# Ryo1011gd/ParticleMethod_FSI

Measured on AMD Instinct MI355X. Metric: particle-steps/sec + achieved HBM GB/s, dam-break, 1/2/4/8 MI355X, higher is better.
Workload: dtype f64; 1 GPU; d1m: 3-D dam break (SURVEY 8d D1M, BASELINE configs[1]), 1397200 particles, ~1397200 per GPU; particles=1397200, dim=3, module=dam, parallelism=single

## Files before the change

### include/mph_gpu.h

```cpp
#ifndef MPH_GPU_H_INCLUDED
#define MPH_GPU_H_INCLUDED

#include <stddef.h>

#ifdef __cplusplus
extern "C" {
#endif

#define MPH_TYPE_COUNT 6
#define MPH_MAX_NEIGHBOR_COUNT 512
#define MPH_ABI_VERSION 6

typedef enum MphModule {
    MPH_MODULE_BAR = 0,
    MPH_MODULE_DAM = 1,
    MPH_MODULE_TUREK_HRON = 2,
    MPH_MODULE_ROLLING1 = 3,
    MPH_MODULE_HYDROELASTIC = 4,
    MPH_MODULE_NONE = 5
} MphModule;

typedef enum MphWallMotion {
    MPH_WALL_RIGID = 0,
    MPH_WALL_ROLLING = 1
// ... 228 lines not shown
    mph_host_exchange_fn host_fn;
    void* host_user;
    int n_glob;
    const int* ids;
    const double* cuts;
} MphSlabOptions;
int mph_create_slab(MphCtx** ctx, const MphConfig* cfg, int n, const int* property, const double* pos,
                    const double* pos0, const double* vel, int device, const MphSlabOptions* opt);
int mph_slab_window(const MphConfig* cfg, int rank, int nranks, int axis, const double* cuts, double* out2);
int mph_dist_selftest(int device);
int mph_dist_info(const MphCtx* ctx, int* out8);
int mph_dist_overlap(const MphCtx* ctx, double* out5);
int mph_list_stats(MphCtx* ctx, double* mean, int* max);
int mph_list_layout(MphCtx* ctx, long long out6[6]);
int mph_idle_wall_stats(MphCtx* ctx, long long out2[2]);
int mph_neighbor_rows(MphCtx* ctx, int first, int count, int* counts, int* ids, long long ids_cap);
int mph_owned_count(const MphCtx* ctx);
int mph_owned_ids(MphCtx* ctx, int* out_ids);
int mph_slab_bounds(const MphConfig* cfg, int rank, int nranks, int axis, const double* cuts, double* out3);
int mph_slab_owner(const MphConfig* cfg, int nranks, int axis, const double* cuts, double c);

#ifdef __cplusplus
}
#endif
#endif
```

### particlemethod_fsi_amd/csrc/mph_ctx.hip

```cpp
#include <hip/hip_runtime.h>

#include <algorithm>
#include <chrono>
#include <cmath>
#include <cstdio>
#include <cstdlib>
#include <cstring>
#include <map>
#include <memory>
#include <string>
#include <vector>

#include "mph_dist.h"
#include "mph_env.h"
#include "mph_rows.h"

using namespace mph;

namespace mph {

int ctx_fail(MphCtx* c, int code, const std::string& msg)
{
    if (c) c->err = msg;
    return code;
// ... 43 lines not shown
    MPH_HIP_OK(c, hipStreamSynchronize(c->stream));
    for (hipGraphExec_t* g : {&c->graph1, &c->graph1t, &c->graph8})
        if (*g) {
            MPH_HIP_OK(c, hipGraphExecDestroy(*g));
            *g = nullptr;
        }
    return MPH_OK;
}

void ctx_fill_launch(MphCtx* c)
{
    Launch& L = c->L;
    set_uniforms(c->P);
    if (env_int("MPH_LIST_FULL", 0) == 1) c->P.rlf = 3.0e38f;
    c->lazy_walls = !c->dist && env_int("MPH_LAZY_WALLS", 1) != 0;
    L.P = &c->P;
    L.stream = c->stream;
    L.xcd_bal_min = env_is("MPH_XCD_BAL_MIN", "") ? (1 << 20) : env_int("MPH_XCD_BAL_MIN", 1 << 20);
    L.S = &c->Sd;
}

int virial_full_lists(MphCtx* c)
{
    if (c->P.rlf >= 3.0e38f) return MPH_OK;
    DevParams Pf = c->P;
    Pf.rlf = 3.0e38f;
    Launch L = c->L;
    L.P = &Pf;
    L.xcd_bal_min = 0x7fffffff;
    launch_neighbors(L);
    MPH_HIP_OK(c, hipGetLastError());
    return MPH_OK;
}
}

namespace {

void enqueue_step(const Launch& L, bool last, hipEvent_t* ev = nullptr)
{
    if (ev) (void)hipEventRecord(ev[0], L.stream);
    Launch La = L;
    La.lazy = !last && L.cmap && !L.mon;
    launch_sort(La, 1);
    if (!last) {
        La.dens_a = La.vstrain = La.divp = nullptr;
        if (!L.P->surface) La.gx = La.gy = La.gz = La.pa = nullptr;
    }
    if (ev) {
        launch_neighbors(La);
        (void)hipEventRecord(ev[1], L.stream);
        launch_pass_a(La);
    } else {
        launch_search_pass_a(La);
    }
    if (last) {
        launch_pass_b(L);
    } else {
// ... 1107 lines not shown
    MPH_HIP_OK(c, hipSetDevice(c->device));
    MPH_HIP_OK(c, hipStreamSynchronize(c->stream));
    unsigned long long steps = 0;
    std::vector<unsigned> seg(kXcdSegs);
    const char* st = reinterpret_cast<const char*>(c->L.st);
    MPH_HIP_OK(c, hipMemcpy(&steps, st + offsetof(DevState, lazy_steps), sizeof(steps), hipMemcpyDeviceToHost));
    MPH_HIP_OK(c, hipMemcpy(seg.data(), st + offsetof(DevState, idle_waves), sizeof(unsigned) * kXcdSegs,
                            hipMemcpyDeviceToHost));
    long long idle = 0;
    for (unsigned v : seg) idle += v;
    out[0] = idle;
    out[1] = (long long)steps;
    return MPH_OK;
}

int mph_neighbor_rows(MphCtx* c, int first, int count, int* counts, int* ids, long long ids_cap)
{
    if (!c || first < 0 || count < 0 || !counts || (!ids && ids_cap > 0)) return MPH_ERR_ARG;
    MPH_CK(ctx_flush(c));
    if (c->dist) return ctx_fail(c, MPH_ERR_UNSUPPORTED, "mph_neighbor_rows: single contexts only");
    if ((long long)first + count > c->n) return ctx_fail(c, MPH_ERR_ARG, "mph_neighbor_rows: range past the particle count");
    if (!count) return 0;
    MPH_HIP_OK(c, hipSetDevice(c->device));
    const int n = c->n;
    if (c->P.rlf < 3.0e38f)
        return ctx_fail(c, MPH_ERR_UNSUPPORTED, "mph_neighbor_rows: the lists keep only the pairs within the passes' "
                                            "radius (create the context with MPH_LIST_FULL=1 for the reference's lists)");
    std::vector<int> id(n), nv(n);
    MPH_HIP_OK(c, hipMemcpy(id.data(), c->L.A.id, sizeof(int) * n, hipMemcpyDeviceToHost));
    MPH_HIP_OK(c, hipMemcpy(nv.data(), c->L.nbcount, sizeof(int) * n, hipMemcpyDeviceToHost));
// ... 240 lines not shown
```

### particlemethod_fsi_amd/csrc/mph_kernels.h

```cpp
#pragma once

#include <hip/hip_runtime.h>

#include "mph_params.h"

namespace mph {

struct StructDev {
    int* orig = nullptr;
    int* slot_of = nullptr;
    int* bidx = nullptr;
    int n_own = 0;
    int n_inner = 0;
    int wo = 0, wi = 0;
    int* ocnt = nullptr;
    int* icnt = nullptr;
    int* eo_nb = nullptr;
    int* ei_nb = nullptr;
    double4* wx0 = nullptr;
    double* L = nullptr;
    double2* lame = nullptr;
    double* inv_rho = nullptr;
    int* clamp = nullptr;
    double4* x0 = nullptr;
// ... 55 lines not shown
    const DevTables* T = nullptr;
    DevState* st = nullptr;
    hipStream_t stream = nullptr;
    Profiler* prof = nullptr;
    Soa A, B;
    int* dst_of = nullptr;
    int *key = nullptr, *slot = nullptr, *tmp = nullptr, *cnt = nullptr, *start = nullptr, *bsum = nullptr;
    int *nbr = nullptr, *ncount = nullptr, *nbcount = nullptr;
    unsigned long long *lhdr = nullptr, *lgap = nullptr;
    int* wface = nullptr;
    VSrc vsrc;
    int xcd_bal_min = 1 << 20;
    unsigned char* cmap = nullptr;
    int cmap_bytes = 0;
    bool lazy = false;
    double *pres = nullptr, *gx = nullptr, *gy = nullptr, *gz = nullptr, *pa = nullptr;
    double *dens_a = nullptr, *vstrain = nullptr, *divp = nullptr;
    double4 *fpart = nullptr;
    double4 *rec = nullptr;
    double4 *force = nullptr, *acc = nullptr;
    const StructDev* S = nullptr;
    const MonitorDev* mon = nullptr;
};

struct SampleDev {
    double origin[3], spacing[3];
    int count[3];
    int tile[3];
    int tiles[3];
    int mask;
// ... 51 lines not shown
```

### particlemethod_fsi_amd/csrc/mph_params.h

```cpp
#pragma once
#include <cmath>

#include <cstddef>
#include <cstdint>

#include "../../include/mph_gpu.h"


namespace mph {

constexpr int kTypes = MPH_TYPE_COUNT;
constexpr int kMaxNeighbor = MPH_MAX_NEIGHBOR_COUNT;
constexpr int kTile = 64;
constexpr int kAlignRows = 128;
constexpr int kMaxJumps = 6;
#ifndef MPH_TILE_EXTRA
#define MPH_TILE_EXTRA kAlignRows
#endif
constexpr int kTileRows = kMaxNeighbor + MPH_TILE_EXTRA;
#ifndef MPH_TILE_PAD
#define MPH_TILE_PAD 1
#endif
constexpr int kTileStride = kTile * (kTileRows + MPH_TILE_PAD);
#if defined(__HIPCC__)
// ... 65 lines not shown
    double ratio[kTypes][kTypes];
    double mu_ij[kTypes][kTypes];
    double cofa[kTypes];
    double mass[kTypes], inv_mass[kTypes], density[kTypes], inv_density[kTypes];
    double bulk[kTypes], bulk_visc[kTypes];
    double wall_rot[kTypes][3][3];
    double wall_omega[kTypes][3];
    double wall_vel[kTypes][3];
    double rc2_lo, rc2_hi;
    double rc2_trim;
    double cwid[3];
    double rg_r2g;
    double cref[3];
    float rc2f_lo, rc2f_hi;
    float rlf;
};

inline void set_uniforms(DevParams& P)
{
    P.rc2_lo = P.rc2 * (1.0 - 1e-10);
    P.rc2_hi = P.rc2 * (1.0 + 1e-10);
    P.rc2_trim = P.rc2 * (1.0 + 4e-6);
    for (int d = 0; d < 3; ++d) P.cwid[d] = 1.0 / P.ginv[d];
    P.rg_r2g = P.rg / P.r2g;
    double hwm = 0.0;
    for (int d = 0; d < 3; ++d) {
        P.cref[d] = P.dmin[d] + P.hw[d];
        hwm = P.hw[d] > hwm ? P.hw[d] : hwm;
    }
    const double rc = std::sqrt(P.rc2);
    const double delta = 2.0 * (2.0 * 1.7320508 * hwm * 1.1920929e-7 / rc) + 4.0e-6;
    P.rc2f_lo = (float)(P.rc2 * (1.0 - delta));
    P.rc2f_hi = (float)(P.rc2 * (1.0 + delta));
    const double rmax = std::fmax(std::fmax(P.ra, P.rg), std::fmax(P.rp, P.rv));
    P.rlf = (float)(rmax * rmax * (1.0 + delta));
}

constexpr int kCoarseShift = 2;
#if defined(__HIPCC__)
__host__ __device__
#endif
constexpr inline int coarse_cells(int g) { return (g + (1 << kCoarseShift) - 1) >> kCoarseShift; }
inline size_t coarse_map_bytes(const int gc[3])
{
    const size_t b = (size_t)coarse_cells(gc[0]) * coarse_cells(gc[1]) * coarse_cells(gc[2]);
    return (b + 15) & ~(size_t)15;
}

constexpr int kXcdSegs = 4096;

struct DevState {
// ... 4 lines not shown
    double wall_rot[kTypes][3][3];
    int overflow;
    int pad0;
    int seam_occ[2];
    int seam_step;
    int seam_pad;
    int seg_work[kXcdSegs];
    int xcd_frac[9];
    int xcd_pad[3];
    unsigned long long lazy_steps;
    unsigned idle_waves[kXcdSegs];
    int seg_lwork[kXcdSegs];
    int seg_swork[kXcdSegs];
    int xcd_sfrac[9];
    int xcd_spad[3];
};
constexpr size_t kStateHead = offsetof(DevState, seg_work);

#if defined(__HIPCC__)
#define MPH_HD __host__ __device__
#else
#define MPH_HD
#endif

MPH_HD inline int jump_count(unsigned long long hdr) { return (int)(hdr >> 56); }
MPH_HD inline int gap_begin(unsigned long long gap, int k) { return (int)((gap >> (8 * k)) & 0xff); }
MPH_HD inline int gap_end(unsigned long long hdr, int k) { return (int)((hdr >> (8 * k)) & 0xff); }

#ifndef MPH_PA_EQR
#define MPH_PA_EQR 1
// ... 74 lines not shown
```

### particlemethod_fsi_amd/csrc/mph_passes.hip

```cpp
#include <cstdio>
#include <cstdlib>
#include <type_traits>

#include "mph_list.h"

namespace mph {

__device__ __forceinline__ void own_velocity(const Soa& A, int i, double& vx, double& vy, double& vz)
{
    const double2 b = A.p6[3 * (size_t)i + 1], c = A.p6[3 * (size_t)i + 2];
    vx = b.y; vy = c.x; vz = c.y;
}


struct PassA {
    double da = 0.0, g0 = 0.0, g1 = 0.0, g2 = 0.0, vs = 0.0, dv = 0.0;
    double s0 = 0.0, s1 = 0.0, s2 = 0.0, v0 = 0.0, v1 = 0.0, v2 = 0.0;
};

template <bool FORCE, bool EQR = false>
__device__ __forceinline__ void pass_a_term(const DevParams& P, const double* s_ratio, const double* s_mu, int ti,
                                            int tj, bool solid, double q0, double q1, double q2, double r2,
                                            double dvx, double dvy, double dvz, PassA& o)
{
#pragma clang fp contract(off)
    double r, ir;
    rsqrt_pair(r2, r, ir);
    const double dot = fma(dvz, q2, fma(dvy, q1, dvx * q0));
    if (EQR) {
        if (r2 <= P.rp2) {
            const double t = r * P.inv_rp;
            const double omt = 1.0 - t;
            const double omt2 = omt * omt;
            const double u = (P.cdp * omt) * ir;
            o.vs = fma(P.cp, omt2, o.vs);
            o.dv = fma(-dot, u, o.dv);
            const bool strict = r2 < P.rp2;
            if (FORCE && strict && !(solid && dev_is_struct(tj))) {
                const double c = u * P.vol;
                o.s0 = fma(c, q0, o.s0);
                o.s1 = fma(c, q1, o.s1);
                o.s2 = fma(c, q2, o.s2);
            }
            if (!solid) {
                const double ratio = s_ratio[ti * kTypes + tj];
                o.da = fma(ratio, (P.ca * t) * omt2, o.da);
                const double w = (ratio * (P.cg * omt2)) * P.rg_r2g;
                o.g0 = fma(q0, w, o.g0);
                o.g1 = fma(q1, w, o.g1);
                o.g2 = fma(q2, w, o.g2);
                if (FORCE && strict) {
                    const double c = ((s_mu[ti * kTypes + tj] * omt) * dot) * ((ir * ir) * ir);
                    o.v0 = fma(c, q0, o.v0);
                    o.v1 = fma(c, q1, o.v1);
                    o.v2 = fma(c, q2, o.v2);
                }
            }
        }
        return;
    }
    if (r2 <= P.rp2) {
        const double omt = 1.0 - r * P.inv_rp;
        const double u = (P.cdp * omt) * ir;
        o.vs = fma(P.cp * omt, omt, o.vs);
        o.dv = fma(-dot, u, o.dv);
        if (FORCE && r2 < P.rp2 && !(solid && dev_is_struct(tj))) {
            const double c = u * P.vol;
            o.s0 = fma(c, q0, o.s0);
            o.s1 = fma(c, q1, o.s1);
            o.s2 = fma(c, q2, o.s2);
        }
    }
    if (!solid) {
        const double ratio = s_ratio[ti * kTypes + tj];
        if (r2 <= P.ra2) {
            const double t = r * P.inv_ra;
            const double omt = 1.0 - t;
            o.da = fma(ratio, ((P.ca * t) * omt) * omt, o.da);
        }
        if (r2 <= P.rg2) {
            const double omt = 1.0 - r * P.inv_rg;
            const double w = (ratio * ((P.cg * omt) * omt)) * P.rg_r2g;
            o.g0 = fma(q0, w, o.g0);
            o.g1 = fma(q1, w, o.g1);
            o.g2 = fma(q2, w, o.g2);
        }
        if (FORCE && r2 < P.rv2) {
            const double c = ((s_mu[ti * kTypes + tj] * (1.0 - r * P.inv_rv)) * dot) * ((ir * ir) * ir);
            o.v0 = fma(c, q0, o.v0);
            o.v1 = fma(c, q1, o.v1);
            o.v2 = fma(c, q2, o.v2);
        }
    }
}

struct PassAOut {
    double *pres, *gx, *gy, *gz, *pa, *dens_a, *vstrain, *divp;
    double4 *fpart, *rec;
};

// ... 38 lines not shown
template <int U, typename Bits>
__device__ __forceinline__ void list_batch(const NbrList& NL, Bits bits_of, int k0, int end,
                                           bool (&ok)[U], int (&jj)[U], int (&TT)[U])
{
    int e[U];
#pragma unroll
    for (int u = 0; u < U; ++u) nbr_at(NL, k0 + u < end ? k0 + u : end - 1, e[u], TT[u]);
    const unsigned bits = bits_of();
#pragma unroll
    for (int u = 0; u < U; ++u) {
        ok[u] = (bits & (1u << u)) != 0;
        jj[u] = e[u];
    }
}

template <bool FAST, int DIM, bool EQR, int U = MPH_UA>
__device__ __forceinline__ void pass_a_loop(const DevParams& P, const double* s_ratio, const double* s_mu,
                                            const Soa& A,
                                            NbrList NL, bool plain, const unsigned* lm, int end, int ti,
                                            bool solid, double xi, double yi, double zi, double vxi, double vyi,
                                            double vzi, PassA& o)
{
    const __amdgpu_buffer_rsrc_t p6r = sized_rsrc(A.p6, (unsigned)P.n * 48u);
    for (int k0 = 0; k0 < end; k0 += U) {
        int jj[U];
        double X[U], Y[U], Z[U], VX[U], VY[U], VZ[U];
        int TT[U];
        bool ok[U];
        list_batch<U>(NL, [&] { return plain ? bit_range(0, end - k0) : row_bits_lds(lm, k0, end); }, k0, end,
                      ok, jj, TT);
#pragma unroll
        for (int u = 0; u < U; ++u) {
            const unsigned off = ok[u] ? (unsigned)jj[u] * 48u : kGatherOob;
            const double2 a = buf_ld16(p6r, off), b = buf_ld16(p6r, off + 16u), c = buf_ld16(p6r, off + 32u);
            X[u] = a.x; Y[u] = a.y; Z[u] = b.x;
            VX[u] = b.y; VY[u] = c.x; VZ[u] = c.y;
        }
#pragma unroll
        for (int u = 0; u < U; ++u) {
            asm volatile("" ::"v"(X[u]), "v"(Y[u]), "v"(Z[u]), "v"(VX[u]), "v"(VY[u]), "v"(VZ[u]));
            if (!ok[u]) continue;
            const double q0 = image_exact<FAST>(X[u] - xi, P.dw[0], P.hw[0], P.w075[0]);
            const double q1 = image_exact<FAST>(Y[u] - yi, P.dw[1], P.hw[1], P.w075[1]);
            const double q2 = image_exact<FAST || DIM == 2>(Z[u] - zi, P.dw[2], P.hw[2], P.w075[2]);
            pass_a_term<true, EQR>(P, s_ratio, s_mu, ti, TT[u], solid, q0, q1, q2, r2_exact(q0, q1, q2),
                                   VX[u] - vxi, VY[u] - vyi, VZ[u] - vzi, o);
        }
    }
}

#ifndef MPH_PA_WPE
#define MPH_PA_WPE 4
#endif
#if MPH_PA_WPE
#define MPH_PA_ATTR __attribute__((amdgpu_waves_per_eu(MPH_PA_WPE)))
#else
#define MPH_PA_ATTR
#endif
template <int DIM>
__global__ __launch_bounds__(MPH_LB) MPH_PA_ATTR void k_pass_a(DevParams P, const DevTables* __restrict__ T, Soa A,
                                                const int* __restrict__ nbr,
                                                const int* __restrict__ ncount,
                                                const unsigned long long* __restrict__ lhdr,
                                                const unsigned long long* __restrict__ lgap, PassAOut pout,
                                                const DevState* __restrict__ st,
                                                unsigned char* __restrict__ cmap, int cmap_bytes)
{
    const int n = dev_n(P);
    if (cmap)
        for (int q = blockIdx.x * MPH_LB + threadIdx.x; q * 16 < cmap_bytes; q += gridDim.x * MPH_LB)
            reinterpret_cast<int4*>(cmap)[q] = make_int4(0, 0, 0, 0);
    const int lb = list_block(st, n, MPH_PASS_A_REV);
    if (lb < 0) return;
    __shared__ double s_ratio[kTypes * kTypes];
    __shared__ double s_mu[kTypes * kTypes];
    if (threadIdx.x < kTypes * kTypes) {
        s_ratio[threadIdx.x] = T->ratio[threadIdx.x];
        s_mu[threadIdx.x] = T->mu_ij[threadIdx.x] * (-P.cvis * P.cdv * P.vol);
    }
    __syncthreads();
    const int i = lb * blockDim.x + threadIdx.x;
    const bool live = i < n;
    const int ii = live ? i : n - 1;
// ... 9 lines not shown
    if (!own) return;
    double vxi, vyi, vzi;
    own_velocity(A, i, vxi, vyi, vzi);
    const int ti = A.type[i];
    const bool solid = dev_is_struct(ti);
    const int end = ncount[i] < kTileRows ? ncount[i] : kTileRows;
    __shared__ unsigned s_mask[kWB][kTile * kMaskWords];
    unsigned* lm = &s_mask[threadIdx.x >> 6][(threadIdx.x & 63) * kMaskWords];
    const unsigned long long hdr = wave_hdr(lhdr, i);
    const bool plain = (hdr >> 56) == 0;
    if (!plain) mask_to_lds(lm, row_mask(hdr, lgap, i, end));
    const NbrList NL = nbr_list(nbr, i);
    PassA o;
    const bool eqr = pass_a_equal_radii(P);
    if (fast && eqr)
        pass_a_loop<true, DIM, true>(P, s_ratio, s_mu, A, NL, plain, lm, end, ti, solid, xi, yi, zi, vxi, vyi, vzi, o);
    else if (fast)
        pass_a_loop<true, DIM, false>(P, s_ratio, s_mu, A, NL, plain, lm, end, ti, solid, xi, yi, zi, vxi, vyi, vzi, o);
    else
        pass_a_loop<false, DIM, false>(P, s_ratio, s_mu, A, NL, plain, lm, end, ti, solid, xi, yi, zi, vxi, vyi, vzi, o);
    pass_a_finish(P, T, ti, i, o, pout, xi, yi, zi);
}


template <bool FAST, bool SURF, int DIM>
__device__ __forceinline__ void pass_b_term(const DevParams& P, const double* s_ratio, const double* gx,
                                            const double* gy, const double* gz, const double* pa, int j, int tj,
                                            double X, double Y, double Z, double PJ, int ti, bool solid,
                                            double xi, double yi, double zi, double gxi, double gyi, double gzi,
                                            double pai, double ai, double dscale, double cpv, double& f0,
                                            double& f1, double& f2)
{
    if (solid && dev_is_struct(tj)) return;
    const double q0 = image_exact<FAST>(X - xi, P.dw[0], P.hw[0], P.w075[0]);
    const double q1 = image_exact<FAST>(Y - yi, P.dw[1], P.hw[1], P.w075[1]);
// ... 260 lines not shown
#pragma unroll
        for (int v = 0; v < 3; ++v) o[3 * u + v] = S[u][v];
    vpres[i] = DIM == 2 ? -1.0 / 2.0 * (S[0][0] + S[1][1]) : -1.0 / 3.0 * (S[0][0] + S[1][1] + S[2][2]);
}


static PassAOut pass_a_out(const Launch& L)
{
    return PassAOut{L.pres, L.gx, L.gy, L.gz, L.pa, L.dens_a, L.vstrain, L.divp, L.fpart, L.rec};
}

void launch_pass_a(const Launch& L)
{
    const DevParams& P = *L.P;
    if (P.n == 0) return;
    by_dim(P.dim, [&](auto D) {
        launch(L.prof, "pass_a", L.stream, k_pass_a<decltype(D)::value>,
               dim3(list_grid(P.n, L.lazy && P.n >= L.xcd_bal_min)), dim3(MPH_LB), P, L.T,
               L.A, L.nbr, L.ncount, L.lhdr, L.lgap, pass_a_out(L), L.st, L.lazy ? L.cmap : nullptr, L.cmap_bytes);
    });
}

void launch_search_pass_a(const Launch& L)
{
    launch_neighbors(L);
    launch_pass_a(L);
}

static StructHook struct_hook(const Launch& L)
{
    StructHook h{};
    if (L.P->n_struct > 0 && L.S && L.S->slot_of) {
        h.slot_of = L.S->slot_of;
        h.sx = L.S->x;
        h.sv = L.S->v;
// ... 40 lines not shown
```

### particlemethod_fsi_amd/csrc/mph_search.hip

```cpp
#include "mph_list.h"

#ifndef MPH_SB
#define MPH_SB 2
#endif
#ifndef MPH_LDS_CAP
#define MPH_LDS_CAP 176
#endif

namespace mph {

__device__ __forceinline__ void start_load2(__amdgpu_buffer_rsrc_t r, unsigned ob, unsigned oe, int& b, int& e)
{
    asm volatile("s_nop 4\n\tbuffer_load_dword %0, %2, %4, 0 offen\n\tbuffer_load_dword %1, %3, %4, 0 offen"
                 : "=&v"(b), "=&v"(e) : "v"(ob), "v"(oe), "s"(r) : "memory");
}
__device__ __forceinline__ void start_landed(int& a, int& b) { asm volatile("" : "+v"(a), "+v"(b)); }

__host__ __device__ constexpr int stage_d(int cap, int sb) { return (cap + sb + 2 + 1) & ~1; }
__host__ __device__ constexpr int stage_t(int cap, int sb) { return (cap + sb + 8 + 3) & ~3; }
__host__ __device__ constexpr int stage_words(int cap, int sb) { return 3 * stage_d(cap, sb) + stage_t(cap, sb) / 2; }


template <int DIM, int PERM> struct CellAxes {
    static constexpr int A0 = DIM == 3 ? order_axis(PERM, 0) : 0;
// ... 99 lines not shown
                    const double q0 = image_exact<false>(xs[u] - xi, P.dw[0], P.hw[0], P.w075[0]);
                    const double q1 = image_exact<false>(ys[u] - yi, P.dw[1], P.hw[1], P.w075[1]);
                    const double q2 = image_exact<DIM == 2>(zs[u] - zi, P.dw[2], P.hw[2], P.w075[2]);
                    const bool a = r2_exact(q0, q1, q2) <= P.rc2;
                    if (a && j < je && j != i) {
                        if (cnt < kMaxNeighbor) out[ell_slot(cnt, 0)] = nbr_entry(j, A.type[j]);
                        ++cnt;
                    }
                }
            }
        }
    }
    return cnt;
}

template <int DIM, int PERM, int SB = MPH_SB, int CAP = MPH_LDS_CAP>
__device__ __forceinline__ int scan_candidates_lds(const DevParams& P, const Soa& A, const int* start,
                                                   int i, bool act, double xi, double yi, double zi,
                                                   int cx, int cy, int cz, int* out, double* sx, int* stored,
                                                   unsigned long long* lgap, unsigned long long* lhdr)
{
    constexpr int kCap32 = stage_words(CAP, SB) / 2 - SB - 1;
    const int lane = threadIdx.x & 63;
    const unsigned long long tb = (unsigned long long)(out - lane);
    const unsigned tlo = __builtin_amdgcn_readfirstlane((unsigned)tb);
    const unsigned thi = __builtin_amdgcn_readfirstlane((unsigned)(tb >> 32));
    const __amdgpu_buffer_rsrc_t tile_rsrc = __builtin_amdgcn_make_buffer_rsrc(
        reinterpret_cast<void*>(((unsigned long long)thi << 32) | tlo), 0, kTile * kTileRows * (int)sizeof(int),
        0x00020000);
    const double lo2 = P.rc2_lo, hi2 = P.rc2_hi;
    using X = CellAxes<DIM, PERM>;
    constexpr int NCOL = DIM == 3 ? kGroups * kGroups : kGroups;
    const int cc[3] = {cx, cy, cz};
    const int cca = cc[X::A2];
    const double cw0 = P.cwid[X::A0], cw1 = P.cwid[X::A1];
    const double uu[3] = {grid_offset(xi, P.corg[0], P.dw[0]), grid_offset(yi, P.corg[1], P.dw[1]),
                          DIM == 3 ? grid_offset(zi, P.corg[2], P.dw[2]) : 0.0};
    const double ua = uu[X::A2];
    const double ginva = P.ginv[X::A2];
    constexpr float kDn = 1.0f - 1.0f / (1 << 20), kUp = 1.0f + 1.0f / (1 << 19);
    constexpr float kBias = 32.0f;
    const float rcm2f = act ? (float)P.rc2_trim * kUp : -1.0f;
    float gx2f = 0.0f;
    const int c0l = cc[X::A0], c1l = DIM == 3 ? cc[X::A1] : 0;
    const float cw0f = (float)cw0, cw1f = (float)cw1;
    const float f0 = (float)(uu[X::A0] - c0l * cw0), f1 = DIM == 3 ? (float)(uu[X::A1] - c1l * cw1) : 0.0f;
    const float mu0 = cw0f * (1.0f / (1 << 20)), mu1 = cw1f * (1.0f / (1 << 20));
    const float g0p = f0 + mu0, g0m = (cw0f - f0) + mu0, g1p = f1 + mu1, g1m = (cw1f - f1) + mu1;
    const float ginvaf = (float)ginva;
    const float caf = (float)(ua * ginva - (double)cca);
    const float cal = (caf - 1e-3f) + kBias, cah = (caf + 1e-3f) + kBias;
    const float rgf = kUp * ginvaf;
    const int rowbase = (DIM == 3 ? (c0l * P.gc[X::A1] + c1l) * P.gc[X::A2] : c0l * P.gc[1]) + cca - (int)kBias;
    const int sa = P.sa;
    const __amdgpu_buffer_rsrc_t srs = arr_rsrc(start);
    auto gap32 = [](int d, float cwf, float gp, float gm) {
        if (d == 0) return 0.0f;
// ... 113 lines not shown
            const float lof = P.rc2f_lo, hif = P.rc2f_hi;
            auto test32 = [&](auto self_tag) {
                constexpr bool SELF = decltype(self_tag)::value;
                for (int j0 = jb; j0 < je; j0 += SB) {
                    float4 r[SB];
#pragma unroll
                    for (int u = 0; u < SB; ++u) r[u] = s4[j0 - lbase + u];
#pragma unroll
                    for (int u = 0; u < SB; ++u) {
                        const int j = j0 + u;
                        const float dx = r[u].x - xf, dy = r[u].y - yf, dz = r[u].z - zf;
                        const float r2f = fmaf(dx, dx, fmaf(dy, dy, dz * dz));
                        bool live = true;
                        if (u > 0) live = j < je;
                        if (SELF) live = live & (j != i);
                        const bool le_lo = r2f <= lof, le_hi = r2f <= hif;
                        bool a = live & le_lo;
                        const unsigned long long mband = __builtin_amdgcn_ballot_w64(le_hi) &
                                                         ~__builtin_amdgcn_ballot_w64(le_lo) &
                                                         __builtin_amdgcn_ballot_w64(live);
                        if (mband) {
                            if (__builtin_amdgcn_inverse_ballot_w64(mband)) {
                                int jj = j;
                                asm volatile("" : "+v"(jj));
                                const double ddx = A.x[jj] - xi, ddy = A.y[jj] - yi, ddz = A.z[jj] - zi;
                                const double r2a = fma(ddx, ddx, fma(ddy, ddy, ddz * ddz));
                                const bool in = r2a <= lo2;
                                a = in;
                                if ((r2a <= hi2) != in) a = accept_band(P, ddx, ddy, ddz);
                            }
// ... 47 lines not shown
    return soff_total(soff);
}

__device__ __forceinline__ void slab_wave_flag(const DevParams& P, const Soa& A, int i, int n, int* wface)
{
    if (P.slab_axis < 0 || !wface) return;
    const bool live = i < n;
    const int ii = live ? i : n - 1;
    const bool own = live && A.id[ii] >= 0;
    const double c = P.slab_axis == 0 ? A.x[ii] : (P.slab_axis == 1 ? A.y[ii] : A.z[ii]);
    const bool inner = c - P.slab_lo > P.slab_h && P.slab_hi - c > P.slab_h;
    const bool face = !__all(!own || inner);
    if ((threadIdx.x & 63) == 0) wface[i >> 6] = face ? 1 : 0;
}

template <int DIM>
__device__ __forceinline__ bool wave_idle_walls(const DevParams& P, const Soa& A, const unsigned char* cmap,
                                                DevState* st, int* ncount, int* nbcount,
                                                unsigned long long* lhdr, int i, int n)
{
    static_assert(kContigReach <= kReach, "the box is widened by kReach on every axis");
    static_assert(2 * kReach < 2 << kCoarseShift, "a lane's box spans at most 3 coarse cells per axis");
    const int tile = __builtin_amdgcn_readfirstlane(i >> 6);
    if (tile * kTile >= n) return false;
    const bool live = i < n;
    int ii = live ? i : n - 1;
    asm volatile("" : "+v"(ii));
    if (!__all(!live || dev_is_wall(A.type[ii]))) return false;
    const double xi = A.x[ii], yi = A.y[ii], zi = A.z[ii];
    if (!wave_search_interior(P, st, live, xi, yi, zi)) return false;
    const int cx = cell_axis(xi, P.corg[0], P.dw[0], P.ginv[0], P.gc[0]);
// ... 3 lines not shown
    const int ay = max(cy - kReach, 0) >> kCoarseShift, by = min(cy + kReach, P.gc[1] - 1) >> kCoarseShift;
    const int az = DIM == 3 ? max(cz - kReach, 0) >> kCoarseShift : 0;
    const int bz = DIM == 3 ? min(cz + kReach, P.gc[2] - 1) >> kCoarseShift : 0;
    const int ny = coarse_cells(P.gc[1]), nz = coarse_cells(P.gc[2]);
    int hit = 0;
#pragma unroll 1
    for (int kx = 0; kx < 3; ++kx) {
#pragma unroll 1
        for (int ky = 0; ky < 3; ++ky) {
            const unsigned char* row = cmap + (min(ax + kx, bx) * ny + min(ay + ky, by)) * nz;
            hit |= row[az] | row[min(az + 1, bz)] | row[bz];
        }
    }
    if (__ballot(hit != 0)) return false;
    if (live) ncount[i] = 0;
    if (live) nbcount[i] = 0;
    if ((threadIdx.x & 63) == 0) {
        lhdr[tile] = 0;
        atomicAdd(&st->idle_waves[(int)(((long long)tile * kXcdSegs) / ((n + 63) >> 6))], 1u);
    }
    return true;
}

template <int DIM, int PERM>
__device__ __forceinline__ int neighbors_body(const DevParams& P, const Soa& A, const int* start, int* nbr,
                                               int* ncount, int* nbcount, unsigned long long* lhdr,
                                               unsigned long long* lgap, DevState* st, double* stage, int i)
{
    const int n = dev_n(P);
    const bool live = i < n;
    const int ii = live ? i : n - 1;
    const int tile = __builtin_amdgcn_readfirstlane(i >> 6);
    if (tile * kTile >= n) return 0;
    if (wave_all_ghosts(P, A, live, ii)) {
        if (live) ncount[i] = 0;
        if (live) nbcount[i] = 0;
        if ((threadIdx.x & 63) == 0) lhdr[tile] = 0;
        return 0;
    }
    const bool own = live && !(P.slab_axis >= 0 && A.id[ii] < 0);
    const double xi = A.x[ii], yi = A.y[ii], zi = A.z[ii];
    const bool fast = wave_search_interior(P, st, own, xi, yi, zi);
    int cnt = 0, stored = 0;
    const int cx = cell_axis(xi, P.corg[0], P.dw[0], P.ginv[0], P.gc[0]);
    const int cy = cell_axis(yi, P.corg[1], P.dw[1], P.ginv[1], P.gc[1]);
    const int cz = DIM == 3 ? cell_axis(zi, P.corg[2], P.dw[2], P.ginv[2], P.gc[2]) : 0;
    int* out = nbr + (size_t)(i >> 6) * kTileStride + (i & 63);
    if (fast) {
        cnt = scan_candidates_lds<DIM, PERM>(P, A, start, i, own, xi, yi, zi, cx, cy, cz, out, stage, &stored,
                                             lgap, lhdr);
    } else {
        if (own)
            cnt = scan_candidates<DIM, PERM>(P, A, start, i, xi, yi, zi, cx, cy, cz, out);
        stored = cnt;
        if ((threadIdx.x & 63) == 0) lhdr[tile] = 0;
    }
    if (live) ncount[i] = stored;
    if (live) nbcount[i] = cnt;
    if (cnt > kMaxNeighbor) atomicOr(&st->overflow, 1);
    return stored;
}

#ifndef MPH_NB_WPE
#define MPH_NB_WPE 8
#endif
template <int DIM, int PERM, bool LAZY>
__global__ __launch_bounds__(MPH_LB) __attribute__((amdgpu_waves_per_eu(MPH_NB_WPE))) void k_neighbors(
    DevParams P, Soa A, const int* __restrict__ start, int* __restrict__ nbr, int* __restrict__ ncount,
    int* __restrict__ nbcount, unsigned long long* __restrict__ lhdr, unsigned long long* __restrict__ lgap,
    DevState* __restrict__ st, int* __restrict__ wface, int bal, const unsigned char* __restrict__ cmap_arg)
{
    const unsigned char* cmap = LAZY ? cmap_arg : nullptr;
    const int n = dev_n(P);
    if (cmap && blockIdx.x == 0 && threadIdx.x == 0) st->lazy_steps += 1;
    int tb;
    if (cmap && bal) {
        tb = list_block(st->xcd_sfrac, n);
        if (tb < 0) return;
    } else {
        if ((int)blockIdx.x >= list_blocks(n)) return;
        tb = xcd_block(blockIdx.x, list_blocks(n));
    }
    __shared__ __attribute__((aligned(16))) double stage[kWB][stage_words(MPH_LDS_CAP, MPH_SB)];
    const int i = tb * blockDim.x + threadIdx.x;
    slab_wave_flag(P, A, i, n, wface);
    const bool idle = cmap && wave_idle_walls<DIM>(P, A, cmap, st, ncount, nbcount, lhdr, i, n);
    const int cnt = idle ? 0
                         : neighbors_body<DIM, PERM>(P, A, start, nbr, ncount, nbcount, lhdr, lgap, st,
                                                     stage[__builtin_amdgcn_readfirstlane(threadIdx.x >> 6)], i);
    if (bal) {
        if (cmap) add_wave_work(st->seg_lwork, cnt, i, n, st->seg_swork, idle);
        else add_wave_work(st->seg_work, cnt, i, n);
    }
}


void launch_neighbors(const Launch& L)
{
    const DevParams& P = *L.P;
    if (P.n == 0) return;
    const int bal = P.n >= L.xcd_bal_min;
    const bool lazy = L.lazy && L.cmap;
    by_dim(P.dim, [&](auto D) {
        constexpr int DIM = decltype(D)::value;
        auto go = [&](auto PERM) {
            if (lazy)
                launch(L.prof, "neighbors", L.stream, k_neighbors<DIM, decltype(PERM)::value, true>,
                       dim3(bal ? list_grid(P.n, true) : blocks(P.n, MPH_LB)), dim3(MPH_LB), P, L.A, L.start, L.nbr,
                       L.ncount, L.nbcount, L.lhdr, L.lgap, L.st, L.wface, bal, L.cmap);
            else
                launch(L.prof, "neighbors", L.stream, k_neighbors<DIM, decltype(PERM)::value, false>,
                       dim3(blocks(P.n, MPH_LB)), dim3(MPH_LB), P, L.A, L.start, L.nbr, L.ncount, L.nbcount, L.lhdr,
                       L.lgap, L.st, L.wface, bal, nullptr);
        };
        if constexpr (DIM == 3) {
            switch (P.perm) {
            case 1: go(Int<1>{}); break;
            case 2: go(Int<2>{}); break;
            case 3: go(Int<3>{}); break;
            case 4: go(Int<4>{}); break;
            default: go(Int<0>{}); break;
// ... 9 lines not shown
```

### particlemethod_fsi_amd/solver.py

```python
from __future__ import annotations

import ctypes
import os
import subprocess

import numpy as np

from . import mphio

PKG_DIR = os.path.dirname(os.path.abspath(__file__))
LIB_DIR = os.path.join(PKG_DIR, "lib")
LIB_PATH = os.environ.get("MPH_GPU_LIB") or os.path.join(LIB_DIR, "libmph_gpu.so")
CSRC_DIR = os.path.join(PKG_DIR, "csrc")

FIELDS = {
    "Position": (0, 3, np.float64), "InitialPosition": (1, 3, np.float64),
    "Velocity": (2, 3, np.float64), "Force": (3, 3, np.float64),
    "Acceleration": (4, 3, np.float64), "GravityCenter": (5, 3, np.float64),
    "PressureP": (6, 1, np.float64), "PressureA": (7, 1, np.float64),
    "DensityA": (8, 1, np.float64), "VolStrainP": (9, 1, np.float64),
    "DivergenceP": (10, 1, np.float64), "Mass": (11, 1, np.float64), "Kappa": (12, 1, np.float64),
    "Lambda": (13, 1, np.float64), "Mu": (14, 1, np.float64),
    "NeighborCount": (15, 1, np.int32), "InitialStructureNeighborCount": (16, 1, np.int32),
    "Property": (17, 1, np.int32), "DeformGradient": (18, 9, np.float64),
# ... 11 lines not shown
EXPORTED_SYMBOLS = [
    "mph_config_default", "mph_read_data_file", "mph_read_grid_header", "mph_read_grid_particles",
    "mph_write_prof_arrays", "mph_write_vtk_arrays", "mph_create", "mph_step", "mph_synchronize",
    "mph_get", "mph_set", "mph_particle_count", "mph_time", "mph_get_scalars", "mph_write_prof",
    "mph_write_vtk", "mph_last_error", "mph_destroy", "mph_profile_steps", "mph_profile_graphs", "mph_neighbor_stats",
    "mph_dist_unique_id", "mph_create_dist", "mph_owned_count", "mph_derive_scalars",
    "mph_structure_init", "mph_create_dist_host", "mph_owned_ids", "mph_slab_bounds",
    "mph_slab_owner", "mph_dist_selftest", "mph_compute_virial",
    "mph_config_sizeof", "mph_write_vtk_async", "mph_output_wait", "mph_write_grid_binary",
    "mph_write_vtu_arrays", "mph_write_vtu", "mph_velocity_profile_arrays",
    "mph_set_initial_velocity_profile", "mph_dist_info", "mph_create_slab", "mph_slab_window",
    "mph_list_stats", "mph_abi_version", "mph_phase_timing", "mph_phase_times",
    "mph_set_step_batching", "mph_neighbor_rows", "mph_dist_overlap", "mph_list_layout",
    "mph_monitor_configure", "mph_monitor_sample_doubles", "mph_monitor_read",
    "mph_sample_grid", "mph_sample_grid_timed", "mph_write_vti_arrays", "mph_idle_wall_stats",
]

ABI_VERSION = 6

HOST_EXCHANGE_FN = ctypes.CFUNCTYPE(ctypes.c_int, ctypes.c_void_p, ctypes.c_void_p, ctypes.c_size_t,
                                    ctypes.c_void_p, ctypes.c_size_t, ctypes.c_void_p, ctypes.c_size_t,
                                    ctypes.c_void_p, ctypes.c_size_t)


class MphSlabOptions(ctypes.Structure):
    _fields_ = [("rank", ctypes.c_int), ("nranks", ctypes.c_int), ("axis", ctypes.c_int),
                ("unique_id128", ctypes.c_char_p), ("host_fn", HOST_EXCHANGE_FN),
                ("host_user", ctypes.c_void_p), ("n_glob", ctypes.c_int), ("ids", ctypes.c_void_p),
                ("cuts", ctypes.c_void_p)]

# ... 121 lines not shown
        "mph_create_slab": (ip, [ctypes.POINTER(vp), cfgp, ip, vp, vp, vp, vp, ip, ctypes.POINTER(MphSlabOptions)]),
        "mph_slab_window": (ip, [cfgp, ip, ip, ip, vp, vp]),
        "mph_phase_timing": (ip, [vp, ip]),
        "mph_phase_times": (ip, [vp, vp]),
        "mph_set_step_batching": (ip, [vp, ip]),
        "mph_neighbor_rows": (ip, [vp, ip, ip, vp, vp, ctypes.c_longlong]),
        "mph_dist_overlap": (ip, [vp, vp]),
        "mph_list_layout": (ip, [vp, vp]),
        "mph_monitor_configure": (ip, [vp, ctypes.POINTER(MphMonitorConfig)]),
        "mph_monitor_sample_doubles": (ip, [vp]),
        "mph_monitor_read": (ctypes.c_longlong, [vp, vp, ctypes.c_longlong, ctypes.POINTER(ctypes.c_longlong)]),
        "mph_sample_grid": (ip, [vp, ctypes.POINTER(MphSampleGrid), vp]),
        "mph_sample_grid_timed": (ip, [vp, ctypes.POINTER(MphSampleGrid), vp, ctypes.POINTER(ctypes.c_double), vp]),
        "mph_write_vti_arrays": (ip, [ctypes.c_char_p, ctypes.POINTER(MphSampleGrid), vp]),
        "mph_idle_wall_stats": (ip, [vp, vp]),
    }
    optional = {"mph_phase_timing", "mph_phase_times", "mph_set_step_batching", "mph_neighbor_rows",
                "mph_dist_overlap", "mph_profile_graphs", "mph_list_stats", "mph_list_layout",
                "mph_monitor_configure", "mph_monitor_sample_doubles", "mph_monitor_read",
                "mph_sample_grid", "mph_sample_grid_timed", "mph_write_vti_arrays", "mph_idle_wall_stats"}
    for name, (res, args) in sig.items():
        if name in optional and not hasattr(L, name):
            continue
        f = getattr(L, name)
        f.restype = res
        f.argtypes = args
    accept = {ABI_VERSION} | {int(v) for v in os.environ.get("MPH_ABI_ACCEPT", "").split(",") if v.strip()}
    if L.mph_abi_version() not in accept:
        raise ImportError("%s has C ABI version %d, these bindings expect %d (rebuild the library)"
                          % (LIB_PATH, L.mph_abi_version(), ABI_VERSION))
    if L.mph_config_sizeof() != ctypes.sizeof(mphio.MphConfig):
        raise ImportError("MphConfig layout mismatch between %s and mphio.MphConfig" % LIB_PATH)
    _lib = L
    return L

# ... 322 lines not shown
        _check(self._L.mph_list_stats(self._h, ctypes.byref(m), ctypes.byref(x)), self._h)
        return m.value, x.value

    def list_layout(self) -> dict:
        a = np.zeros(6, np.int64)
        _check(self._L.mph_list_layout(self._h, a.ctypes.data), self._h)
        keys = ["waves", "waves_jumped", "jumps", "max_jumps", "gap_rows", "max_rows"]
        return {k: int(v) for k, v in zip(keys, a)}

    def idle_wall_stats(self) -> dict:
        a = np.zeros(2, np.int64)
        if hasattr(self._L, "mph_idle_wall_stats"):
            _check(self._L.mph_idle_wall_stats(self._h, a.ctypes.data), self._h)
        return {"idle_wave_steps": int(a[0]), "lazy_steps": int(a[1])}

    def neighbor_rows(self, first: int = 0, count: int | None = None):
        if count is None:
            count = self.n - first
        counts = np.zeros(count, np.int32)
        cap = max(1, count * 128)
        while True:
            ids = np.zeros(cap, np.int32)
            r = self._L.mph_neighbor_rows(self._h, int(first), int(count), counts.ctypes.data, ids.ctypes.data, cap)
            need = int(np.minimum(counts, 512).sum()) if r == -1 else 0
            if r == -1 and need > cap:
                cap = need
                continue
            _check(r, self._h)
            break
        offsets = np.concatenate([[0], np.cumsum(np.minimum(counts, 512))]).astype(np.int64)
# ... 41 lines not shown
```

Baseline: 1.434 billion particle-steps/s.

## Add lean lazy steps that skip unused density/gradient terms and trim search radius

On lazy, non-final steps the pass-A kernel gets a LEAN variant that skips the density and gradient accumulations. Those outputs are already nulled on such steps. The neighbor search gets a matching LEAN variant that uses a tighter float cutoff (rl_trimf), keeps only pairs within rlf without the banded lo/hi classification, and skips writing nbcount. The aim is to cut arithmetic and list-building work on intermediate steps. It adds template instantiations, a device counter for lean steps and a stats API, and it relies on the lean search condition (rlf <= rc2f_lo) holding for correctness.

```diff
diff --git a/include/mph_gpu.h b/include/mph_gpu.h
--- a/include/mph_gpu.h
+++ b/include/mph_gpu.h
@@ -266,6 +266,7 @@
 int mph_list_stats(MphCtx* ctx, double* mean, int* max);
 int mph_list_layout(MphCtx* ctx, long long out6[6]);
 int mph_idle_wall_stats(MphCtx* ctx, long long out2[2]);
+int mph_lean_step_stats(MphCtx* ctx, long long out2[2]);
 int mph_neighbor_rows(MphCtx* ctx, int first, int count, int* counts, int* ids, long long ids_cap);
 int mph_owned_count(const MphCtx* ctx);
 int mph_owned_ids(MphCtx* ctx, int* out_ids);
diff --git a/particlemethod_fsi_amd/csrc/mph_ctx.hip b/particlemethod_fsi_amd/csrc/mph_ctx.hip
--- a/particlemethod_fsi_amd/csrc/mph_ctx.hip
+++ b/particlemethod_fsi_amd/csrc/mph_ctx.hip
@@ -81,6 +81,8 @@
     set_uniforms(c->P);
     if (env_int("MPH_LIST_FULL", 0) == 1) c->P.rlf = 3.0e38f;
     c->lazy_walls = !c->dist && env_int("MPH_LAZY_WALLS", 1) != 0;
+    L.lean_ok = env_int("MPH_LEAN_STEPS", 1) != 0;
+    L.lean_search = L.lean_ok && lean_search_ok(c->P);
     L.P = &c->P;
     L.stream = c->stream;
     L.xcd_bal_min = env_is("MPH_XCD_BAL_MIN", "") ? (1 << 20) : env_int("MPH_XCD_BAL_MIN", 1 << 20);
@@ -108,6 +110,7 @@
     if (ev) (void)hipEventRecord(ev[0], L.stream);
     Launch La = L;
     La.lazy = !last && L.cmap && !L.mon;
+    La.lean = La.lazy && L.lean_ok;
     launch_sort(La, 1);
     if (!last) {
         La.dens_a = La.vstrain = La.divp = nullptr;
@@ -1245,6 +1248,22 @@
     return MPH_OK;
 }
 
+int mph_lean_step_stats(MphCtx* c, long long out[2])
+{
+    if (!c || !out) return MPH_ERR_ARG;
+    MPH_CK(ctx_flush(c));
+    MPH_HIP_OK(c, hipSetDevice(c->device));
+    MPH_HIP_OK(c, hipStreamSynchronize(c->stream));
+    unsigned long long steps[2] = {0, 0};
+    static_assert(offsetof(DevState, lean_pass_a_steps) == offsetof(DevState, lean_search_steps) + sizeof(steps[0]),
+                  "the two counters are read in one copy");
+    MPH_HIP_OK(c, hipMemcpy(steps, reinterpret_cast<const char*>(c->L.st) + offsetof(DevState, lean_search_steps),
+                            sizeof(steps), hipMemcpyDeviceToHost));
+    out[0] = (long long)steps[0];
+    out[1] = (long long)steps[1];
+    return MPH_OK;
+}
+
 int mph_neighbor_rows(MphCtx* c, int first, int count, int* counts, int* ids, long long ids_cap)
 {
     if (!c || first < 0 || count < 0 || !counts || (!ids && ids_cap > 0)) return MPH_ERR_ARG;
diff --git a/particlemethod_fsi_amd/csrc/mph_kernels.h b/particlemethod_fsi_amd/csrc/mph_kernels.h
--- a/particlemethod_fsi_amd/csrc/mph_kernels.h
+++ b/particlemethod_fsi_amd/csrc/mph_kernels.h
@@ -93,6 +93,7 @@
     unsigned char* cmap = nullptr;
     int cmap_bytes = 0;
     bool lazy = false;
+    bool lean_ok = false, lean_search = false, lean = false;
     double *pres = nullptr, *gx = nullptr, *gy = nullptr, *gz = nullptr, *pa = nullptr;
     double *dens_a = nullptr, *vstrain = nullptr, *divp = nullptr;
     double4 *fpart = nullptr;
diff --git a/particlemethod_fsi_amd/csrc/mph_params.h b/particlemethod_fsi_amd/csrc/mph_params.h
--- a/particlemethod_fsi_amd/csrc/mph_params.h
+++ b/particlemethod_fsi_amd/csrc/mph_params.h
@@ -103,7 +103,11 @@
     double cref[3];
     float rc2f_lo, rc2f_hi;
     float rlf;
-};
+    float rl_trimf;
+};
+static_assert(offsetof(DevParams, rl_trimf) == offsetof(DevParams, rlf) + sizeof(float) &&
+              offsetof(DevParams, rl_trimf) + sizeof(float) == sizeof(DevParams),
+              "rl_trimf fills the tail padding behind rlf: the size is the one without it");
 
 inline void set_uniforms(DevParams& P)
 {
@@ -123,7 +127,11 @@
     P.rc2f_hi = (float)(P.rc2 * (1.0 + delta));
     const double rmax = std::fmax(std::fmax(P.ra, P.rg), std::fmax(P.rp, P.rv));
     P.rlf = (float)(rmax * rmax * (1.0 + delta));
-}
+    const double d1 = 1.0 + delta;
+    P.rl_trimf = (float)std::fmin(rmax * rmax * d1 * d1 * d1 * (1.0 + 4e-6), P.rc2_trim);
+}
+
+inline bool lean_search_ok(const DevParams& P) { return P.rlf <= P.rc2f_lo; }
 
 constexpr int kCoarseShift = 2;
 #if defined(__HIPCC__)
@@ -158,6 +166,7 @@
     int seg_swork[kXcdSegs];
     int xcd_sfrac[9];
     int xcd_spad[3];
+    unsigned long long lean_search_steps, lean_pass_a_steps;
 };
 constexpr size_t kStateHead = offsetof(DevState, seg_work);
 
diff --git a/particlemethod_fsi_amd/csrc/mph_passes.hip b/particlemethod_fsi_amd/csrc/mph_passes.hip
--- a/particlemethod_fsi_amd/csrc/mph_passes.hip
+++ b/particlemethod_fsi_amd/csrc/mph_passes.hip
@@ -18,7 +18,7 @@
     double s0 = 0.0, s1 = 0.0, s2 = 0.0, v0 = 0.0, v1 = 0.0, v2 = 0.0;
 };
 
-template <bool FORCE, bool EQR = false>
+template <bool FORCE, bool EQR = false, bool LEAN = false>
 __device__ __forceinline__ void pass_a_term(const DevParams& P, const double* s_ratio, const double* s_mu, int ti,
                                             int tj, bool solid, double q0, double q1, double q2, double r2,
                                             double dvx, double dvy, double dvz, PassA& o)
@@ -43,12 +43,14 @@
                 o.s2 = fma(c, q2, o.s2);
             }
             if (!solid) {
-                const double ratio = s_ratio[ti * kTypes + tj];
-                o.da = fma(ratio, (P.ca * t) * omt2, o.da);
-                const double w = (ratio * (P.cg * omt2)) * P.rg_r2g;
-                o.g0 = fma(q0, w, o.g0);
-                o.g1 = fma(q1, w, o.g1);
-                o.g2 = fma(q2, w, o.g2);
+                if (!LEAN) {
+                    const double ratio = s_ratio[ti * kTypes + tj];
+                    o.da = fma(ratio, (P.ca * t) * omt2, o.da);
+                    const double w = (ratio * (P.cg * omt2)) * P.rg_r2g;
+                    o.g0 = fma(q0, w, o.g0);
+                    o.g1 = fma(q1, w, o.g1);
+                    o.g2 = fma(q2, w, o.g2);
+                }
                 if (FORCE && strict) {
                     const double c = ((s_mu[ti * kTypes + tj] * omt) * dot) * ((ir * ir) * ir);
                     o.v0 = fma(c, q0, o.v0);
@@ -72,18 +74,20 @@
         }
     }
     if (!solid) {
-        const double ratio = s_ratio[ti * kTypes + tj];
-        if (r2 <= P.ra2) {
-            const double t = r * P.inv_ra;
-            const double omt = 1.0 - t;
-            o.da = fma(ratio, ((P.ca * t) * omt) * omt, o.da);
-        }
-        if (r2 <= P.rg2) {
-            const double omt = 1.0 - r * P.inv_rg;
-            const double w = (ratio * ((P.cg * omt) * omt)) * P.rg_r2g;
-            o.g0 = fma(q0, w, o.g0);
-            o.g1 = fma(q1, w, o.g1);
-            o.g2 = fma(q2, w, o.g2);
+        if (!LEAN) {
+            const double ratio = s_ratio[ti * kTypes + tj];
+            if (r2 <= P.ra2) {
+                const double t = r * P.inv_ra;
+                const double omt = 1.0 - t;
+                o.da = fma(ratio, ((P.ca * t) * omt) * omt, o.da);
+            }
+            if (r2 <= P.rg2) {
+                const double omt = 1.0 - r * P.inv_rg;
+                const double w = (ratio * ((P.cg * omt) * omt)) * P.rg_r2g;
+                o.g0 = fma(q0, w, o.g0);
+                o.g1 = fma(q1, w, o.g1);
+                o.g2 = fma(q2, w, o.g2);
+            }
         }
         if (FORCE && r2 < P.rv2) {
             const double c = ((s_mu[ti * kTypes + tj] * (1.0 - r * P.inv_rv)) * dot) * ((ir * ir) * ir);
@@ -152,7 +156,7 @@
     }
 }
 
-template <bool FAST, int DIM, bool EQR, int U = MPH_UA>
+template <bool FAST, int DIM, bool EQR, bool LEAN, int U = MPH_UA>
 __device__ __forceinline__ void pass_a_loop(const DevParams& P, const double* s_ratio, const double* s_mu,
                                             const Soa& A,
                                             NbrList NL, bool plain, const unsigned* lm, int end, int ti,
@@ -181,8 +185,8 @@
             const double q0 = image_exact<FAST>(X[u] - xi, P.dw[0], P.hw[0], P.w075[0]);
             const double q1 = image_exact<FAST>(Y[u] - yi, P.dw[1], P.hw[1], P.w075[1]);
             const double q2 = image_exact<FAST || DIM == 2>(Z[u] - zi, P.dw[2], P.hw[2], P.w075[2]);
-            pass_a_term<true, EQR>(P, s_ratio, s_mu, ti, TT[u], solid, q0, q1, q2, r2_exact(q0, q1, q2),
-                                   VX[u] - vxi, VY[u] - vyi, VZ[u] - vzi, o);
+            pass_a_term<true, EQR, LEAN>(P, s_ratio, s_mu, ti, TT[u], solid, q0, q1, q2, r2_exact(q0, q1, q2),
+                                         VX[u] - vxi, VY[u] - vyi, VZ[u] - vzi, o);
         }
     }
 }
@@ -195,7 +199,7 @@
 #else
 #define MPH_PA_ATTR
 #endif
-template <int DIM>
+template <int DIM, bool LEAN = false>
 __global__ __launch_bounds__(MPH_LB) MPH_PA_ATTR void k_pass_a(DevParams P, const DevTables* __restrict__ T, Soa A,
                                                 const int* __restrict__ nbr,
                                                 const int* __restrict__ ncount,
@@ -205,6 +209,7 @@
                                                 unsigned char* __restrict__ cmap, int cmap_bytes)
 {
     const int n = dev_n(P);
+    if (LEAN && blockIdx.x == 0 && threadIdx.x == 0) const_cast<DevState*>(st)->lean_pass_a_steps += 1;
     if (cmap)
         for (int q = blockIdx.x * MPH_LB + threadIdx.x; q * 16 < cmap_bytes; q += gridDim.x * MPH_LB)
             reinterpret_cast<int4*>(cmap)[q] = make_int4(0, 0, 0, 0);
@@ -244,11 +249,14 @@
     PassA o;
     const bool eqr = pass_a_equal_radii(P);
     if (fast && eqr)
-        pass_a_loop<true, DIM, true>(P, s_ratio, s_mu, A, NL, plain, lm, end, ti, solid, xi, yi, zi, vxi, vyi, vzi, o);
+        pass_a_loop<true, DIM, true, LEAN>(P, s_ratio, s_mu, A, NL, plain, lm, end, ti, solid, xi, yi, zi, vxi, vyi,
+                                           vzi, o);
     else if (fast)
-        pass_a_loop<true, DIM, false>(P, s_ratio, s_mu, A, NL, plain, lm, end, ti, solid, xi, yi, zi, vxi, vyi, vzi, o);
+        pass_a_loop<true, DIM, false, LEAN>(P, s_ratio, s_mu, A, NL, plain, lm, end, ti, solid, xi, yi, zi, vxi, vyi,
+                                            vzi, o);
     else
-        pass_a_loop<false, DIM, false>(P, s_ratio, s_mu, A, NL, plain, lm, end, ti, solid, xi, yi, zi, vxi, vyi, vzi, o);
+        pass_a_loop<false, DIM, false, LEAN>(P, s_ratio, s_mu, A, NL, plain, lm, end, ti, solid, xi, yi, zi, vxi, vyi,
+                                             vzi, o);
     pass_a_finish(P, T, ti, i, o, pout, xi, yi, zi);
 }
 
@@ -539,11 +547,16 @@
 {
     const DevParams& P = *L.P;
     if (P.n == 0) return;
-    by_dim(P.dim, [&](auto D) {
-        launch(L.prof, "pass_a", L.stream, k_pass_a<decltype(D)::value>,
-               dim3(list_grid(P.n, L.lazy && P.n >= L.xcd_bal_min)), dim3(MPH_LB), P, L.T,
-               L.A, L.nbr, L.ncount, L.lhdr, L.lgap, pass_a_out(L), L.st, L.lazy ? L.cmap : nullptr, L.cmap_bytes);
-    });
+    const bool lean = L.lean && L.lazy && !L.gx && !L.dens_a;
+    auto go = [&](auto LEAN) {
+        by_dim(P.dim, [&](auto D) {
+            launch(L.prof, "pass_a", L.stream, k_pass_a<decltype(D)::value, decltype(LEAN)::value>,
+                   dim3(list_grid(P.n, L.lazy && P.n >= L.xcd_bal_min)), dim3(MPH_LB), P, L.T, L.A, L.nbr, L.ncount,
+                   L.lhdr, L.lgap, pass_a_out(L), L.st, L.lazy ? L.cmap : nullptr, L.cmap_bytes);
+        });
+    };
+    if (lean) go(std::true_type{});
+    else go(std::false_type{});
 }
 
 void launch_search_pass_a(const Launch& L)
diff --git a/particlemethod_fsi_amd/csrc/mph_search.hip b/particlemethod_fsi_amd/csrc/mph_search.hip
--- a/particlemethod_fsi_amd/csrc/mph_search.hip
+++ b/particlemethod_fsi_amd/csrc/mph_search.hip
@@ -137,7 +137,7 @@
     return cnt;
 }
 
-template <int DIM, int PERM, int SB = MPH_SB, int CAP = MPH_LDS_CAP>
+template <int DIM, int PERM, bool LEAN, int SB = MPH_SB, int CAP = MPH_LDS_CAP>
 __device__ __forceinline__ int scan_candidates_lds(const DevParams& P, const Soa& A, const int* start,
                                                    int i, bool act, double xi, double yi, double zi,
                                                    int cx, int cy, int cz, int* out, double* sx, int* stored,
@@ -163,7 +163,7 @@
     const double ginva = P.ginv[X::A2];
     constexpr float kDn = 1.0f - 1.0f / (1 << 20), kUp = 1.0f + 1.0f / (1 << 19);
     constexpr float kBias = 32.0f;
-    const float rcm2f = act ? (float)P.rc2_trim * kUp : -1.0f;
+    const float rcm2f = act ? (LEAN ? P.rl_trimf : (float)P.rc2_trim) * kUp : -1.0f;
     float gx2f = 0.0f;
     const int c0l = cc[X::A0], c1l = DIM == 3 ? cc[X::A1] : 0;
     const float cw0f = (float)cw0, cw1f = (float)cw1;
@@ -307,6 +307,14 @@
                         bool live = true;
                         if (u > 0) live = j < je;
                         if (SELF) live = live & (j != i);
+                        if constexpr (LEAN) {
+                            if (live & (r2f <= P.rlf)) {
+                                __builtin_amdgcn_raw_buffer_store_b32(nbr_entry(j, __float_as_int(r[u].w)), tile_rsrc,
+                                                                      soff & kSoffMask, 0, 0);
+                                soff += kListKeep;
+                            }
+                            continue;
+                        }
                         const bool le_lo = r2f <= lof, le_hi = r2f <= hif;
                         bool a = live & le_lo;
                         const unsigned long long mband = __builtin_amdgcn_ballot_w64(le_hi) &
@@ -384,7 +392,7 @@
     if ((threadIdx.x & 63) == 0) wface[i >> 6] = face ? 1 : 0;
 }
 
-template <int DIM>
+template <int DIM, bool LEAN>
 __device__ __forceinline__ bool wave_idle_walls(const DevParams& P, const Soa& A, const unsigned char* cmap,
                                                 DevState* st, int* ncount, int* nbcount,
                                                 unsigned long long* lhdr, int i, int n)
@@ -418,7 +426,7 @@
     }
     if (__ballot(hit != 0)) return false;
     if (live) ncount[i] = 0;
-    if (live) nbcount[i] = 0;
+    if (!LEAN && live) nbcount[i] = 0;
     if ((threadIdx.x & 63) == 0) {
         lhdr[tile] = 0;
         atomicAdd(&st->idle_waves[(int)(((long long)tile * kXcdSegs) / ((n + 63) >> 6))], 1u);
@@ -426,7 +434,7 @@
     return true;
 }
 
-template <int DIM, int PERM>
+template <int DIM, int PERM, bool LEAN>
 __device__ __forceinline__ int neighbors_body(const DevParams& P, const Soa& A, const int* start, int* nbr,
                                                int* ncount, int* nbcount, unsigned long long* lhdr,
                                                unsigned long long* lgap, DevState* st, double* stage, int i)
@@ -451,7 +459,7 @@
     const int cz = DIM == 3 ? cell_axis(zi, P.corg[2], P.dw[2], P.ginv[2], P.gc[2]) : 0;
     int* out = nbr + (size_t)(i >> 6) * kTileStride + (i & 63);
     if (fast) {
-        cnt = scan_candidates_lds<DIM, PERM>(P, A, start, i, own, xi, yi, zi, cx, cy, cz, out, stage, &stored,
+        cnt = scan_candidates_lds<DIM, PERM, LEAN>(P, A, start, i, own, xi, yi, zi, cx, cy, cz, out, stage, &stored,
                                              lgap, lhdr);
     } else {
         if (own)
@@ -460,7 +468,7 @@
         if ((threadIdx.x & 63) == 0) lhdr[tile] = 0;
     }
     if (live) ncount[i] = stored;
-    if (live) nbcount[i] = cnt;
+    if (!LEAN && live) nbcount[i] = cnt;
     if (cnt > kMaxNeighbor) atomicOr(&st->overflow, 1);
     return stored;
 }
@@ -468,7 +476,7 @@
 #ifndef MPH_NB_WPE
 #define MPH_NB_WPE 8
 #endif
-template <int DIM, int PERM, bool LAZY>
+template <int DIM, int PERM, bool LAZY, bool LEAN = false>
 __global__ __launch_bounds__(MPH_LB) __attribute__((amdgpu_waves_per_eu(MPH_NB_WPE))) void k_neighbors(
     DevParams P, Soa A, const int* __restrict__ start, int* __restrict__ nbr, int* __restrict__ ncount,
     int* __restrict__ nbcount, unsigned long long* __restrict__ lhdr, unsigned long long* __restrict__ lgap,
@@ -476,7 +484,11 @@
 {
     const unsigned char* cmap = LAZY ? cmap_arg : nullptr;
     const int n = dev_n(P);
-    if (cmap && blockIdx.x == 0 && threadIdx.x == 0) st->lazy_steps += 1;
+    static_assert(LAZY || !LEAN, "only a lazy step is lean");
+    if (cmap && blockIdx.x == 0 && threadIdx.x == 0) {
+        st->lazy_steps += 1;
+        if (LEAN) st->lean_search_steps += 1;
+    }
     int tb;
     if (cmap && bal) {
         tb = list_block(st->xcd_sfrac, n);
@@ -488,9 +500,9 @@
     __shared__ __attribute__((aligned(16))) double stage[kWB][stage_words(MPH_LDS_CAP, MPH_SB)];
     const int i = tb * blockDim.x + threadIdx.x;
     slab_wave_flag(P, A, i, n, wface);
-    const bool idle = cmap && wave_idle_walls<DIM>(P, A, cmap, st, ncount, nbcount, lhdr, i, n);
+    const bool idle = cmap && wave_idle_walls<DIM, LEAN>(P, A, cmap, st, ncount, nbcount, lhdr, i, n);
     const int cnt = idle ? 0
-                         : neighbors_body<DIM, PERM>(P, A, start, nbr, ncount, nbcount, lhdr, lgap, st,
+                         : neighbors_body<DIM, PERM, LEAN>(P, A, start, nbr, ncount, nbcount, lhdr, lgap, st,
                                                      stage[__builtin_amdgcn_readfirstlane(threadIdx.x >> 6)], i);
     if (bal) {
         if (cmap) add_wave_work(st->seg_lwork, cnt, i, n, st->seg_swork, idle);
@@ -505,10 +517,15 @@
     if (P.n == 0) return;
     const int bal = P.n >= L.xcd_bal_min;
     const bool lazy = L.lazy && L.cmap;
+    const bool lean = lazy && L.lean && L.lean_search && lean_search_ok(P);
     by_dim(P.dim, [&](auto D) {
         constexpr int DIM = decltype(D)::value;
         auto go = [&](auto PERM) {
-            if (lazy)
+            if (lean)
+                launch(L.prof, "neighbors", L.stream, k_neighbors<DIM, decltype(PERM)::value, true, true>,
+                       dim3(bal ? list_grid(P.n, true) : blocks(P.n, MPH_LB)), dim3(MPH_LB), P, L.A, L.start, L.nbr,
+                       L.ncount, L.nbcount, L.lhdr, L.lgap, L.st, L.wface, bal, L.cmap);
+            else if (lazy)
                 launch(L.prof, "neighbors", L.stream, k_neighbors<DIM, decltype(PERM)::value, true>,
                        dim3(bal ? list_grid(P.n, true) : blocks(P.n, MPH_LB)), dim3(MPH_LB), P, L.A, L.start, L.nbr,
                        L.ncount, L.nbcount, L.lhdr, L.lgap, L.st, L.wface, bal, L.cmap);
diff --git a/particlemethod_fsi_amd/solver.py b/particlemethod_fsi_amd/solver.py
--- a/particlemethod_fsi_amd/solver.py
+++ b/particlemethod_fsi_amd/solver.py
@@ -49,6 +49,7 @@
     "mph_set_step_batching", "mph_neighbor_rows", "mph_dist_overlap", "mph_list_layout",
     "mph_monitor_configure", "mph_monitor_sample_doubles", "mph_monitor_read",
     "mph_sample_grid", "mph_sample_grid_timed", "mph_write_vti_arrays", "mph_idle_wall_stats",
+    "mph_lean_step_stats",
 ]
 
 ABI_VERSION = 6
@@ -200,11 +201,13 @@
         "mph_sample_grid_timed": (ip, [vp, ctypes.POINTER(MphSampleGrid), vp, ctypes.POINTER(ctypes.c_double), vp]),
         "mph_write_vti_arrays": (ip, [ctypes.c_char_p, ctypes.POINTER(MphSampleGrid), vp]),
         "mph_idle_wall_stats": (ip, [vp, vp]),
+        "mph_lean_step_stats": (ip, [vp, vp]),
     }
     optional = {"mph_phase_timing", "mph_phase_times", "mph_set_step_batching", "mph_neighbor_rows",
                 "mph_dist_overlap", "mph_profile_graphs", "mph_list_stats", "mph_list_layout",
                 "mph_monitor_configure", "mph_monitor_sample_doubles", "mph_monitor_read",
-                "mph_sample_grid", "mph_sample_grid_timed", "mph_write_vti_arrays", "mph_idle_wall_stats"}
+                "mph_sample_grid", "mph_sample_grid_timed", "mph_write_vti_arrays", "mph_idle_wall_stats",
+                "mph_lean_step_stats"}
     for name, (res, args) in sig.items():
         if name in optional and not hasattr(L, name):
             continue
@@ -557,6 +560,12 @@
             _check(self._L.mph_idle_wall_stats(self._h, a.ctypes.data), self._h)
         return {"idle_wave_steps": int(a[0]), "lazy_steps": int(a[1])}
 
+    def lean_step_stats(self) -> dict:
+        a = np.zeros(2, np.int64)
+        if hasattr(self._L, "mph_lean_step_stats"):
+            _check(self._L.mph_lean_step_stats(self._h, a.ctypes.data), self._h)
+        return {"search_steps": int(a[0]), "pass_a_steps": int(a[1])}
+
     def neighbor_rows(self, first: int = 0, count: int | None = None):
         if count is None:
             count = self.n - first
```

Measured after the change: 1.474 billion particle-steps/s (median of 6 runs). +2.8%, better.
